# eth-cscs/conflux

Hardware: NVIDIA H100
Metric: LU GFLOP/s (FP64, (2/3)N^3) (higher is better)
Workload: dtype f64

## Files before the change

conflux_b200/csrc/common.cuh:

```cuda
#pragma once
#include <cuda_runtime.h>

#include "../../include/conflux_b200.h"

#include <cstdint>
#include <cstdio>

namespace cflx {

void set_last_error(const char* fmt, ...);

#define CFLX_CUDA(call)                                                                                \
    do {                                                                                               \
        cudaError_t e__ = (call);                                                                      \
        if (e__ != cudaSuccess) {                                                                      \
            ::cflx::set_last_error("%s:%d: %s -> %s", __FILE__, __LINE__, #call, cudaGetErrorString(e__)); \
            return CFLX_ERR_CUDA;                                                              \
        }                                                                                              \
    } while (0)

#define CFLX_TRY(call)              \
    do {                            \
        int rc__ = (call);          \
        if (rc__ != 0) return rc__; \
    } while (0)

static inline int64_t round_up(int64_t x, int64_t m) { return (x + m - 1) / m * m; }

struct DevBuf {
    void* p = nullptr;
    DevBuf() = default;
    DevBuf(const DevBuf&) = delete;
    DevBuf& operator=(const DevBuf&) = delete;
    ~DevBuf() { cudaFree(p); }
    int alloc(size_t bytes) {
        CFLX_CUDA(cudaMalloc(&p, bytes + 4096));
        return CFLX_OK;
    }
    template <class T>
    T* as() { return (T*)p; }
};
template <int N>
struct Events {
    cudaEvent_t e[N] = {};
    Events() = default;
    Events(const Events&) = delete;
    Events& operator=(const Events&) = delete;
    ~Events() {
        for (cudaEvent_t x : e)
            if (x) cudaEventDestroy(x);
    }
    int create() {
        for (cudaEvent_t& x : e) CFLX_CUDA(cudaEventCreate(&x));
        return CFLX_OK;
    }
    cudaEvent_t operator[](int i) const { return e[i]; }
};

struct PerDeviceMax {
    size_t v[64] = {0};
    bool raise(size_t want) {
        int dev = 0;
        cudaGetDevice(&dev);
        dev &= 63;
        if (want > v[dev]) {
            v[dev] = want;
            return true;
        }
        return false;
    }
};

#ifdef __CUDACC__
__device__ __forceinline__ uint32_t smem_u32(const void* p) { return (uint32_t)__cvta_generic_to_shared(p); }

__device__ __forceinline__ void mbar_init(uint64_t* bar, uint32_t count) {
    asm volatile("mbarrier.init.shared::cta.b64 [%0], %1;" ::"r"(smem_u32(bar)), "r"(count));
}
__device__ __forceinline__ void fence_barrier_init() { asm volatile("fence.mbarrier_init.release.cluster;" ::: "memory"); }
__device__ __forceinline__ void fence_proxy_async() { asm volatile("fence.proxy.async.shared::cta;" ::: "memory"); }
__device__ __forceinline__ void mbar_arrive_expect_tx(uint64_t* bar, uint32_t bytes) {
    asm volatile("mbarrier.arrive.expect_tx.shared::cta.b64 _, [%0], %1;" ::"r"(smem_u32(bar)), "r"(bytes) : "memory");
}
__device__ __forceinline__ void mbar_arrive(uint64_t* bar) {
    asm volatile("mbarrier.arrive.shared::cta.b64 _, [%0];" ::"r"(smem_u32(bar)) : "memory");
}
__device__ __forceinline__ void mbar_wait(uint64_t* bar, uint32_t parity) {
    asm volatile(
        "{\n\t.reg .pred p;\n\t"
        "WAIT_%=:\n\t"
        "mbarrier.try_wait.parity.shared::cta.b64 p, [%0], %1;\n\t"
        "@p bra DONE_%=;\n\t"
        "bra WAIT_%=;\n\t"
        "DONE_%=:\n\t}" ::"r"(smem_u32(bar)),
        "r"(parity)
        : "memory");
}
__device__ __forceinline__ bool mbar_test(uint64_t* bar, uint32_t parity) {
    uint32_t ok;
    asm volatile(
        "{\n\t.reg .pred p;\n\t"
        "mbarrier.test_wait.parity.shared::cta.b64 p, [%1], %2;\n\t"
        "selp.u32 %0, 1, 0, p;\n\t}"
        : "=r"(ok)
        : "r"(smem_u32(bar)), "r"(parity)
        : "memory");
    return ok != 0;
}
__device__ __forceinline__ void bulk_g2s(void* smem_dst, const void* gsrc, uint32_t bytes, uint64_t* bar) {
    asm volatile("cp.async.bulk.shared::cluster.global.mbarrier::complete_tx::bytes [%0], [%1], %2, [%3];" ::"r"(
                     smem_u32(smem_dst)),
                 "l"(gsrc), "r"(bytes), "r"(smem_u32(bar))
                 : "memory");
}

__device__ __forceinline__ void dmma884(double& c0, double& c1, double a, double b) {
    asm volatile("mma.sync.aligned.m8n8k4.row.col.f64.f64.f64.f64 {%0,%1}, {%2}, {%3}, {%0,%1};"
                 : "+d"(c0), "+d"(c1)
                 : "d"(a), "d"(b));
}

__device__ __forceinline__ void dmma16x8x4(double (&c)[4], const double (&a)[2], double b) {
    asm("mma.sync.aligned.m16n8k4.row.col.f64.f64.f64.f64 {%0,%1,%2,%3}, {%4,%5}, {%6}, {%0,%1,%2,%3};"
        : "+d"(c[0]), "+d"(c[1]), "+d"(c[2]), "+d"(c[3])
        : "d"(a[0]), "d"(a[1]), "d"(b));
}
__device__ __forceinline__ void dmma16x8x8(double (&c)[4], const double (&a)[4], const double (&b)[2]) {
    asm("mma.sync.aligned.m16n8k8.row.col.f64.f64.f64.f64 {%0,%1,%2,%3}, {%4,%5,%6,%7}, {%8,%9}, {%0,%1,%2,%3};"
        : "+d"(c[0]), "+d"(c[1]), "+d"(c[2]), "+d"(c[3])
        : "d"(a[0]), "d"(a[1]), "d"(a[2]), "d"(a[3]), "d"(b[0]), "d"(b[1]));
}
__device__ __forceinline__ void dmma16x8x16(double (&c)[4], const double (&a)[8], const double (&b)[4]) {
    asm("mma.sync.aligned.m16n8k16.row.col.f64.f64.f64.f64 {%0,%1,%2,%3}, {%4,%5,%6,%7,%8,%9,%10,%11}, "
        "{%12,%13,%14,%15}, {%0,%1,%2,%3};"
        : "+d"(c[0]), "+d"(c[1]), "+d"(c[2]), "+d"(c[3])
        : "d"(a[0]), "d"(a[1]), "d"(a[2]), "d"(a[3]), "d"(a[4]), "d"(a[5]), "d"(a[6]), "d"(a[7]), "d"(b[0]),
          "d"(b[1]), "d"(b[2]), "d"(b[3]));
}

__device__ __forceinline__ int ld_acquire_gpu(const int* p) {
    int v;
    asm volatile("ld.acquire.gpu.global.b32 %0, [%1];" : "=r"(v) : "l"(p) : "memory");
    return v;
}
__device__ __forceinline__ void st_release_gpu(int* p, int v) {
    asm volatile("st.release.gpu.global.b32 [%0], %1;" ::"l"(p), "r"(v) : "memory");
}
__device__ __forceinline__ double ld_cg_f64(const double* p) {
    double v;
    asm volatile("ld.global.cg.f64 %0, [%1];" : "=d"(v) : "l"(p) : "memory");
    return v;
}
__device__ __forceinline__ int ld_cg_s32(const int* p) {
    int v;
    asm volatile("ld.global.cg.s32 %0, [%1];" : "=r"(v) : "l"(p) : "memory");
    return v;
}
#endif

}
```

conflux_b200/csrc/gemm.cu:

```cuda
#include <cstdlib>

#include "common.cuh"
#include "kernels.h"

namespace cflx {

namespace {
constexpr int BK = 16, STAGES = 4;

template <int WM, int WN>
struct Cfg {
    static constexpr int BM = 64 * WM, BN = 32 * WN;
    static constexpr int LDA = BM + 4, LDB = BN + 4;
    static constexpr int NCONS = WM * WN, NTHREADS = (NCONS + 1) * 32;
    static constexpr bool STAGE_C = (WM == 2);
    static constexpr int NBAR = 2 * STAGES + (STAGE_C ? WM * STAGES : 0);
    static constexpr size_t SMEM = (size_t)STAGES * BK * (LDA + LDB) * sizeof(double) + NBAR * sizeof(uint64_t);
    static_assert(!STAGE_C || (LDA == LDB && 64 / 16 == STAGES), "one slab per warp row and stage, in both parts");
};

__device__ __forceinline__ double2 ld_c2(const double* p) {
    double2 v;
    asm("ld.global.v2.f64 {%0, %1}, [%2];" : "=d"(v.x), "=d"(v.y) : "l"(p));
    return v;
}

template <int WM, int WN, int MINB>
__global__ void __launch_bounds__(Cfg<WM, WN>::NTHREADS, MINB) gemm_tn_kernel(GemmArgs g) {
    using C = Cfg<WM, WN>;
    constexpr int BM = C::BM, BN = C::BN, LDA = C::LDA, LDB = C::LDB, NCONS = C::NCONS;
    extern __shared__ __align__(128) unsigned char smem_raw[];
    double* sA = reinterpret_cast<double*>(smem_raw);
    double* sB = sA + STAGES * BK * LDA;
    uint64_t* full = reinterpret_cast<uint64_t*>(sB + STAGES * BK * LDB);
    uint64_t* empty = full + STAGES;
    uint64_t* cfull = empty + STAGES;

    const int warp = threadIdx.x >> 5, lane = threadIdx.x & 31;
    const int m0 = blockIdx.y * BM, n0 = blockIdx.x * BN;

    if (threadIdx.x == 0) {
        for (int s = 0; s < STAGES; ++s) {
            mbar_init(&full[s], 1);
            mbar_init(&empty[s], NCONS);
        }
        if constexpr (C::STAGE_C)
            for (int b = 0; b < WM * STAGES; ++b) mbar_init(&cfull[b], 1);
        fence_barrier_init();
    }
    __syncthreads();

    if (warp == NCONS) {
        int wm = g.M - m0;
        wm = wm > BM ? BM : ((wm + 1) & ~1);
        int wn = g.N - n0;
        wn = wn > BN ? BN : ((wn + 1) & ~1);
        const int rr = lane & 15;
        const int nkt = (g.K + BK - 1) / BK;
        const bool use_c = (g.beta != 0.0);
        for (int kt = 0; kt < nkt; ++kt) {
            const int s = kt % STAGES, u = kt / STAGES;
            if (u > 0) mbar_wait(&empty[s], (u - 1) & 1);
            const int rows = min(BK, g.K - kt * BK);
            if (lane == 0) mbar_arrive_expect_tx(&full[s], (uint32_t)(rows * (wm + wn) * sizeof(double)));
            __syncwarp();
            if (rr < rows) {
                const int64_t k = (int64_t)kt * BK + rr;
                if (lane < 16)
                    bulk_g2s(sA + (s * BK + rr) * LDA, g.AT + k * g.ldat + m0, (uint32_t)(wm * sizeof(double)), &full[s]);
                else
                    bulk_g2s(sB + (s * BK + rr) * LDB, g.B + k * g.ldb + n0, (uint32_t)(wn * sizeof(double)), &full[s]);
            }
        }
        if constexpr (C::STAGE_C) {
            if (use_c)
                for (int i = 0; i < STAGES; ++i) {
                    const int s = (nkt + i) % STAGES, kt = nkt + i - STAGES;
                    if (kt >= 0) mbar_wait(&empty[s], (kt / STAGES) & 1);
                    const int wr = lane >> 4, r0 = m0 + 64 * wr + 16 * i;
                    const int rows = max(0, min(16, g.M - r0));
                    uint64_t* bar = &cfull[wr * STAGES + i];
                    if (rr == 0) mbar_arrive_expect_tx(bar, (uint32_t)(rows * wn * sizeof(double)));
                    __syncwarp();
                    if (rr < rows)
                        bulk_g2s(sA + (wr * STAGES + s) * BK * LDA + rr * LDA + 4 * (rr & 1),
                                 g.C + (int64_t)(r0 + rr) * g.ldc + n0, (uint32_t)(wn * sizeof(double)), bar);
                }
        }
        return;
    }

    const int wm_off = (warp / WN) * 64, wn_off = (warp % WN) * 32;
    const int g4 = lane >> 2, t4 = lane & 3;
    double acc[4][4][4];
#pragma unroll
    for (int i = 0; i < 4; ++i)
#pragma unroll
        for (int j = 0; j < 4; ++j) acc[i][j][0] = acc[i][j][1] = acc[i][j][2] = acc[i][j][3] = 0.0;

    int kt = 0;
    for (; kt * BK < g.K; ++kt) {
        const int s = kt % STAGES, u = kt / STAGES;
        mbar_wait(&full[s], u & 1);
        const double* a_s = sA + s * BK * LDA + wm_off + g4;
        const double* b_s = sB + s * BK * LDB + wn_off + g4;
        const int rows = min(BK, g.K - kt * BK);
#pragma unroll
        for (int kk = 0; kk < BK; kk += 8) {
            if (kk < rows) {
                const bool hi = kk + 4 < rows;
                const double* a_k = a_s + (kk + t4) * LDA;
                const double* b_k = b_s + (kk + t4) * LDB;
                double b[4][2];
#pragma unroll
                for (int j = 0; j < 4; ++j) {
                    b[j][0] = b_k[8 * j];
                    b[j][1] = hi ? b_k[4 * LDB + 8 * j] : 0.0;
                }
#pragma unroll
                for (int i = 0; i < 4; ++i) {
                    const double a[4] = {a_k[16 * i], a_k[16 * i + 8], hi ? a_k[4 * LDA + 16 * i] : 0.0,
                                         hi ? a_k[4 * LDA + 16 * i + 8] : 0.0};
#pragma unroll
                    for (int j = 0; j < 4; ++j) dmma16x8x8(acc[i][j], a, b[j]);
                }
            }
        }
        __syncwarp();
        if (lane == 0) mbar_arrive(&empty[s]);
    }

    const double alpha = g.alpha, beta = g.beta;
    const bool use_c = (beta != 0.0);
    const int row0 = m0 + wm_off + g4, col0 = n0 + wn_off + 2 * t4;
    if constexpr (C::STAGE_C) {
        const int wr = warp / WN, nkt = kt;
#pragma unroll
        for (int i = 0; i < 4; ++i) {
            const double* cs = sA + (wr * STAGES + (nkt + i) % STAGES) * BK * LDA + 4 * (g4 & 1) + wn_off + 2 * t4;
            if (use_c) mbar_wait(&cfull[wr * STAGES + i], 0);
#pragma unroll
            for (int h = 0; h < 2; ++h) {
                const int row = row0 + 16 * i + 8 * h;
#pragma unroll
                for (int j = 0; j < 4; ++j) {
                    const int col = col0 + 8 * j;
                    if (row < g.M && col < g.N) {
                        double2 cv = make_double2(0.0, 0.0);
                        if (use_c) cv = *reinterpret_cast<const double2*>(cs + (g4 + 8 * h) * LDA + 8 * j);
                        double2 out;
                        out.x = fma(alpha, acc[i][j][2 * h], beta * cv.x);
                        out.y = fma(alpha, acc[i][j][2 * h + 1], beta * cv.y);
                        *reinterpret_cast<double2*>(g.D + (int64_t)row * g.ldd + col) = out;
                    }
                }
            }
        }
    } else {
#pragma unroll
        for (int sl = 0; sl < 8; ++sl) {
            const int row = row0 + 8 * sl;
            double2 cv[4];
#pragma unroll
            for (int j = 0; j < 4; ++j) {
                const int col = col0 + 8 * j;
                cv[j] = make_double2(0.0, 0.0);
                if (use_c && row < g.M && col < g.N) cv[j] = ld_c2(g.C + (int64_t)row * g.ldc + col);
            }
#pragma unroll
            for (int j = 0; j < 4; ++j) {
                const int col = col0 + 8 * j;
                if (row < g.M && col < g.N) {
                    double2 out;
                    out.x = fma(alpha, acc[sl / 2][j][2 * (sl & 1)], beta * cv[j].x);
                    out.y = fma(alpha, acc[sl / 2][j][2 * (sl & 1) + 1], beta * cv[j].y);
                    *reinterpret_cast<double2*>(g.D + (int64_t)row * g.ldd + col) = out;
                }
            }
        }
    }
}
}

namespace {
template <int WM, int WN, int MINB>
int setup_one() {
    static PerDeviceMax cfg;
    if (cfg.raise(Cfg<WM, WN>::SMEM))
        CFLX_CUDA(cudaFuncSetAttribute(gemm_tn_kernel<WM, WN, MINB>, cudaFuncAttributeMaxDynamicSharedMemorySize,
                                       (int)Cfg<WM, WN>::SMEM));
    return CFLX_OK;
}
template <int WM, int WN, int MINB>
int launch_one(const GemmArgs& g, cudaStream_t stream) {
    using C = Cfg<WM, WN>;
    CFLX_TRY((setup_one<WM, WN, MINB>()));
    dim3 grid((g.N + C::BN - 1) / C::BN, (g.M + C::BM - 1) / C::BM);
    gemm_tn_kernel<WM, WN, MINB><<<grid, C::NTHREADS, C::SMEM, stream>>>(g);
    CFLX_CUDA(cudaGetLastError());
    return CFLX_OK;
}
int tile_variant() {
    static int v = -1;
    if (v < 0) {
        const char* e = getenv("CFLX_GEMM_TILE");
        v = (e && atoi(e) == 64) ? 64 : 128;
    }
    return v;
}
}

int gemm_tn_setup() {
    CFLX_TRY((setup_one<2, 4, 1>()));
    CFLX_TRY((setup_one<1, 4, 2>()));
    return CFLX_OK;
}

int launch_gemm_tn(const GemmArgs& g, cudaStream_t stream) {
    if (g.M <= 0 || g.N <= 0 || g.K <= 0) return CFLX_OK;
    if ((g.K & 3) || (g.N & 1) || (g.ldat & 1) || (g.ldb & 1) || (g.ldc & 1) || (g.ldd & 1)) {
        set_last_error("gemm_tn: unsupported shape M=%d N=%d K=%d ld=(%lld,%lld,%lld,%lld)", g.M, g.N, g.K,
                       (long long)g.ldat, (long long)g.ldb, (long long)g.ldc, (long long)g.ldd);
        return CFLX_ERR_UNSUPPORTED;
    }
    if (tile_variant() == 64) return launch_one<1, 4, 2>(g, stream);
    return launch_one<2, 4, 1>(g, stream);
}

}
```

Before: 25170.

## Add warp-specialized GEMM with TMA-bulk epilogue and multi-tile runs per CTA

Adds a new warp-specialized FP64 GEMM kernel. One producer warp streams A/B k-slabs through an mbarrier ring using bulk async copies, eight consumer warps run DMMA with registers raised via setmaxnreg, and a mover warp prefetches C into a shared staging tile and writes D back with bulk shared-to-global copies. Each CTA walks a run of N-tiles so the epilogue of one tile overlaps the next tile's mainloop. The kernel is chosen only when the grid stays large enough relative to the SM count. The trade-off is higher register and shared-memory pressure, with one CTA per SM and only BK=8 slabs per stage.

```diff
diff --git a/conflux_b200/csrc/common.cuh b/conflux_b200/csrc/common.cuh
--- a/conflux_b200/csrc/common.cuh
+++ b/conflux_b200/csrc/common.cuh
@@ -113,6 +113,18 @@
                  "l"(gsrc), "r"(bytes), "r"(smem_u32(bar))
                  : "memory");
 }
+__device__ __forceinline__ void bulk_s2g(void* gdst, const void* smem_src, uint32_t bytes) {
+    asm volatile("cp.async.bulk.global.shared::cta.bulk_group [%0], [%1], %2;" ::"l"(gdst), "r"(smem_u32(smem_src)),
+                 "r"(bytes)
+                 : "memory");
+}
+__device__ __forceinline__ void bulk_commit() { asm volatile("cp.async.bulk.commit_group;" ::: "memory"); }
+__device__ __forceinline__ void bulk_wait_read_all() { asm volatile("cp.async.bulk.wait_group.read 0;" ::: "memory"); }
+
+template <uint32_t R>
+__device__ __forceinline__ void setmaxnreg_inc() { asm volatile("setmaxnreg.inc.sync.aligned.u32 %0;" ::"n"(R)); }
+template <uint32_t R>
+__device__ __forceinline__ void setmaxnreg_dec() { asm volatile("setmaxnreg.dec.sync.aligned.u32 %0;" ::"n"(R)); }
 
 __device__ __forceinline__ void dmma884(double& c0, double& c1, double a, double b) {
     asm volatile("mma.sync.aligned.m8n8k4.row.col.f64.f64.f64.f64 {%0,%1}, {%2}, {%3}, {%0,%1};"
diff --git a/conflux_b200/csrc/gemm.cu b/conflux_b200/csrc/gemm.cu
--- a/conflux_b200/csrc/gemm.cu
+++ b/conflux_b200/csrc/gemm.cu
@@ -180,6 +180,161 @@
         }
     }
 }
+
+namespace ws {
+constexpr int BK = 8, STAGES = 5, BM = 128, BN = 128, LD = 132;
+constexpr int NCONS = 8, NTHREADS = 384, PRODUCER = NCONS, MOVER = NCONS + 1;
+constexpr int RUN_MAX = 8;
+constexpr size_t RING = (size_t)STAGES * BK * 2 * LD * sizeof(double);
+constexpr size_t TILE = (size_t)BM * LD * sizeof(double);
+constexpr int NBAR = 2 * STAGES + 2;
+constexpr size_t SMEM = RING + TILE + NBAR * sizeof(uint64_t);
+static_assert(SMEM <= 227 * 1024, "one CTA per SM");
+__device__ __forceinline__ int srow(int r) { return r * LD + 4 * (r & 1); }
+}
+
+__global__ void __launch_bounds__(ws::NTHREADS, 1) gemm_tn_ws_kernel(GemmArgs g, int run) {
+    constexpr int BK = ws::BK, STAGES = ws::STAGES, BM = ws::BM, BN = ws::BN, LD = ws::LD, NCONS = ws::NCONS;
+    using ws::srow;
+    extern __shared__ __align__(128) unsigned char smem_raw[];
+    double* sA = reinterpret_cast<double*>(smem_raw);
+    double* sB = sA + STAGES * BK * LD;
+    double* sT = sB + STAGES * BK * LD;
+    uint64_t* full = reinterpret_cast<uint64_t*>(sT + BM * LD);
+    uint64_t* empty = full + STAGES;
+    uint64_t* cfull = empty + STAGES;
+    uint64_t* dfull = cfull + 1;
+
+    const int warp = threadIdx.x >> 5, lane = threadIdx.x & 31;
+    const int m0 = blockIdx.y * BM, nt0 = blockIdx.x * run;
+    const int ntiles = min(run, (g.N + BN - 1) / BN - nt0);
+    const int nkt = (g.K + BK - 1) / BK;
+    const bool use_c = (g.beta != 0.0);
+
+    if (threadIdx.x == 0) {
+        for (int s = 0; s < STAGES; ++s) {
+            mbar_init(&full[s], 1);
+            mbar_init(&empty[s], NCONS);
+        }
+        mbar_init(cfull, 1);
+        mbar_init(dfull, NCONS * 32);
+        fence_barrier_init();
+    }
+    __syncthreads();
+
+    if (warp >= NCONS) {
+        setmaxnreg_dec<48>();
+        const int mrows = min(BM, g.M - m0);
+        if (warp == ws::PRODUCER) {
+            const int wm = mrows == BM ? BM : ((mrows + 1) & ~1);
+            const int rr = lane & 15;
+            for (int t = 0, it = 0; t < ntiles; ++t) {
+                const int n0 = (nt0 + t) * BN, wn = min(BN, g.N - n0);
+                for (int kt = 0; kt < nkt; ++kt, ++it) {
+                    const int s = it % STAGES, u = it / STAGES;
+                    if (u > 0) mbar_wait(&empty[s], (u - 1) & 1);
+                    const int rows = min(BK, g.K - kt * BK);
+                    if (lane == 0) mbar_arrive_expect_tx(&full[s], (uint32_t)(rows * (wm + wn) * sizeof(double)));
+                    __syncwarp();
+                    if (rr < rows) {
+                        const int64_t k = (int64_t)kt * BK + rr;
+                        if (lane < 16)
+                            bulk_g2s(sA + (s * BK + rr) * LD, g.AT + k * g.ldat + m0, (uint32_t)(wm * sizeof(double)),
+                                     &full[s]);
+                        else
+                            bulk_g2s(sB + (s * BK + rr) * LD, g.B + k * g.ldb + n0, (uint32_t)(wn * sizeof(double)),
+                                     &full[s]);
+                    }
+                }
+            }
+        } else if (warp == ws::MOVER) {
+            for (int t = 0; t <= ntiles; ++t) {
+                if (t > 0) {
+                    const int n0 = (nt0 + t - 1) * BN, wn = min(BN, g.N - n0);
+                    mbar_wait(dfull, (t - 1) & 1);
+                    for (int r = lane; r < mrows; r += 32)
+                        bulk_s2g(g.D + (int64_t)(m0 + r) * g.ldd + n0, sT + srow(r), (uint32_t)(wn * sizeof(double)));
+                    bulk_commit();
+                    bulk_wait_read_all();
+                }
+                if (t == ntiles) break;
+                if (use_c) {
+                    const int n0 = (nt0 + t) * BN, wn = min(BN, g.N - n0);
+                    if (lane == 0) mbar_arrive_expect_tx(cfull, (uint32_t)(mrows * wn * sizeof(double)));
+                    __syncwarp();
+                    for (int r = lane; r < mrows; r += 32)
+                        bulk_g2s(sT + srow(r), g.C + (int64_t)(m0 + r) * g.ldc + n0, (uint32_t)(wn * sizeof(double)),
+                                 cfull);
+                } else if (lane == 0) {
+                    mbar_arrive(cfull);
+                }
+            }
+        }
+        return;
+    }
+    setmaxnreg_inc<224>();
+
+    const int wm_off = (warp >> 2) * 64, wn_off = (warp & 3) * 32;
+    const int g4 = lane >> 2, t4 = lane & 3;
+    const double alpha = g.alpha, beta = g.beta;
+    for (int t = 0, it = 0; t < ntiles; ++t) {
+        double acc[4][4][4];
+#pragma unroll
+        for (int i = 0; i < 4; ++i)
+#pragma unroll
+            for (int j = 0; j < 4; ++j) acc[i][j][0] = acc[i][j][1] = acc[i][j][2] = acc[i][j][3] = 0.0;
+
+        for (int kt = 0; kt < nkt; ++kt, ++it) {
+            const int s = it % STAGES, u = it / STAGES;
+            mbar_wait(&full[s], u & 1);
+            const int rows = min(BK, g.K - kt * BK);
+#pragma unroll
+            for (int kk = 0; kk < BK; kk += 8) {
+                if (kk < rows) {
+                    const bool hi = kk + 4 < rows;
+                    const double* a_k = sA + (s * BK + kk + t4) * LD + wm_off + g4;
+                    const double* b_k = sB + (s * BK + kk + t4) * LD + wn_off + g4;
+                    double b[4][2];
+#pragma unroll
+                    for (int j = 0; j < 4; ++j) {
+                        b[j][0] = b_k[8 * j];
+                        b[j][1] = hi ? b_k[4 * LD + 8 * j] : 0.0;
+                    }
+#pragma unroll
+                    for (int i = 0; i < 4; ++i) {
+                        const double a[4] = {a_k[16 * i], a_k[16 * i + 8], hi ? a_k[4 * LD + 16 * i] : 0.0,
+                                             hi ? a_k[4 * LD + 16 * i + 8] : 0.0};
+#pragma unroll
+                        for (int j = 0; j < 4; ++j) dmma16x8x8(acc[i][j], a, b[j]);
+                    }
+                }
+            }
+            __syncwarp();
+            if (lane == 0) mbar_arrive(&empty[s]);
+        }
+
+        mbar_wait(cfull, t & 1);
+#pragma unroll
+        for (int i = 0; i < 4; ++i)
+#pragma unroll
+            for (int h = 0; h < 2; ++h) {
+                double* rp = sT + srow(wm_off + 16 * i + 8 * h + g4) + wn_off + 2 * t4;
+#pragma unroll
+                for (int j = 0; j < 4; ++j) {
+                    double2* p = reinterpret_cast<double2*>(rp + 8 * j);
+                    double2 cv = make_double2(0.0, 0.0);
+                    if (use_c) cv = *p;
+                    double2 out;
+                    out.x = fma(alpha, acc[i][j][2 * h], beta * cv.x);
+                    out.y = fma(alpha, acc[i][j][2 * h + 1], beta * cv.y);
+                    *p = out;
+                }
+            }
+        fence_proxy_async();
+        mbar_arrive(dfull);
+    }
+}
+
 }
 
 namespace {
@@ -200,6 +355,36 @@
     CFLX_CUDA(cudaGetLastError());
     return CFLX_OK;
 }
+int setup_ws() {
+    static PerDeviceMax cfg;
+    if (cfg.raise(ws::SMEM))
+        CFLX_CUDA(cudaFuncSetAttribute(gemm_tn_ws_kernel, cudaFuncAttributeMaxDynamicSharedMemorySize, (int)ws::SMEM));
+    return CFLX_OK;
+}
+int sm_count() {
+    static int n[64] = {0};
+    int dev = 0;
+    cudaGetDevice(&dev);
+    dev &= 63;
+    if (n[dev] == 0 && cudaDeviceGetAttribute(&n[dev], cudaDevAttrMultiProcessorCount, dev) != cudaSuccess) n[dev] = 0;
+    return n[dev] > 0 ? n[dev] : 1;
+}
+int forced_run() {
+    static int v = -1;
+    if (v < 0) {
+        const char* e = getenv("CFLX_GEMM_RUN");
+        const int r = e ? atoi(e) : 0;
+        v = (r >= 1 && r <= ws::RUN_MAX) ? r : 0;
+    }
+    return v;
+}
+int pick_run(int ntm, int ntn) {
+    if (forced_run()) return forced_run();
+    const int64_t sms = sm_count();
+    for (int r = 4; r >= 2; --r)
+        if (r <= ntn && (int64_t)ntm * ((ntn + r - 1) / r) >= 2 * sms) return r;
+    return 0;
+}
 int tile_variant() {
     static int v = -1;
     if (v < 0) {
@@ -211,6 +396,7 @@
 }
 
 int gemm_tn_setup() {
+    CFLX_TRY(setup_ws());
     CFLX_TRY((setup_one<2, 4, 1>()));
     CFLX_TRY((setup_one<1, 4, 2>()));
     return CFLX_OK;
@@ -224,7 +410,14 @@
         return CFLX_ERR_UNSUPPORTED;
     }
     if (tile_variant() == 64) return launch_one<1, 4, 2>(g, stream);
-    return launch_one<2, 4, 1>(g, stream);
-}
-
-}
+    const int ntn = (g.N + ws::BN - 1) / ws::BN, ntm = (g.M + ws::BM - 1) / ws::BM;
+    const int run = pick_run(ntm, ntn);
+    if (run == 0) return launch_one<2, 4, 1>(g, stream);
+    CFLX_TRY(setup_ws());
+    dim3 grid((ntn + run - 1) / run, ntm);
+    gemm_tn_ws_kernel<<<grid, ws::NTHREADS, ws::SMEM, stream>>>(g, run);
+    CFLX_CUDA(cudaGetLastError());
+    return CFLX_OK;
+}
+
+}
```

Measured after the change: 25620 (median of 6 runs). +1.8%, better.
